# ueda0319/neddf

Hardware: NVIDIA H100
Metric: ray-samples/s (800x800x192) (higher is better)
Workload: dtype f16x3-split operands, f32 accumulate

## Files before the change

### neddf_b200/csrc/composite.cu

```cuda
#include "common.cuh"

namespace neddf {

constexpr int kWarpsPerBlock = 8;

__global__ void __launch_bounds__(kWarpsPerBlock * 32)
composite_kernel(const float* __restrict__ dists, const float* __restrict__ density,
                 const float* __restrict__ color, const float* __restrict__ penalty, int64_t n_rays,
                 int n_edges, float max_dist, float* __restrict__ weight, float* __restrict__ depth,
                 float* __restrict__ color_out, float* __restrict__ transmittance,
                 float* __restrict__ penalty_out, int* __restrict__ status) {
  const int lane = threadIdx.x & 31;
  const int64_t warp = (int64_t)blockIdx.x * kWarpsPerBlock + (threadIdx.x >> 5);
  const int64_t n_warps = (int64_t)gridDim.x * kWarpsPerBlock;
  const int n_int = n_edges - 1;
  bool saw_nan = false;

  for (int64_t ray = warp; ray < n_rays; ray += n_warps) {
    const float* drow = dists + ray * n_edges;
    const float* srow = density + ray * n_edges;
    const float* crow = color + ray * n_edges * 3;
    const float* prow = penalty ? penalty + ray * n_edges : nullptr;
    float* wrow = weight ? weight + ray * n_int : nullptr;

    double carry = 1.0;
    float acc_d = 0.f, acc_r = 0.f, acc_g = 0.f, acc_b = 0.f, acc_p = 0.f;
    for (int base = 0; base < n_int; base += 32) {
      const int j = base + lane;
      const bool live = j < n_int;
      float dj = 0.f, delta = 0.f, o = 0.f;
      if (live) {
        dj = drow[j];
        delta = drow[j + 1] - dj;
        o = 1.0f - (float)exp((double)(-srow[j] * delta));
      }
      double f = live ? (double)(1.0f - o + 1e-7f) : 1.0;
      double incl = f;
#pragma unroll
      for (int s = 1; s < 32; s <<= 1) {
        double up = __shfl_up_sync(0xffffffffu, incl, s);
        if (lane >= s) incl *= up;
      }
      double excl = __shfl_up_sync(0xffffffffu, incl, 1);
      if (lane == 0) excl = 1.0;
      float t_j = (float)(carry * excl);
      if (live) {
        float w = o * t_j;
        saw_nan |= (w != w);
        if (wrow) wrow[j] = w;
        acc_d += w * dj;
        acc_r += w * crow[3 * j + 0];
        acc_g += w * crow[3 * j + 1];
        acc_b += w * crow[3 * j + 2];
        if (prow) acc_p += delta * prow[j];
      }
      carry = carry * __shfl_sync(0xffffffffu, incl, 31);
    }
#pragma unroll
    for (int s = 16; s > 0; s >>= 1) {
      acc_d += __shfl_xor_sync(0xffffffffu, acc_d, s);
      acc_r += __shfl_xor_sync(0xffffffffu, acc_r, s);
      acc_g += __shfl_xor_sync(0xffffffffu, acc_g, s);
      acc_b += __shfl_xor_sync(0xffffffffu, acc_b, s);
      acc_p += __shfl_xor_sync(0xffffffffu, acc_p, s);
    }
    if (lane == 0) {
      float t_last = (float)carry;
      if (depth) depth[ray] = acc_d + t_last * max_dist;
      if (color_out) {
        color_out[3 * ray + 0] = acc_r;
        color_out[3 * ray + 1] = acc_g;
        color_out[3 * ray + 2] = acc_b;
      }
      if (transmittance) transmittance[ray] = t_last;
      if (penalty_out) penalty_out[ray] = acc_p;
    }
  }
  if (status && __any_sync(0xffffffffu, saw_nan) && lane == 0) atomicOr(status, 1);
}

__global__ void __launch_bounds__(kWarpsPerBlock * 32)
composite_backward_kernel(const float* __restrict__ dists, const float* __restrict__ density,
                          const float* __restrict__ color, int64_t n_rays, int n_edges, float max_dist,
                          const float* __restrict__ g_weight, const float* __restrict__ g_depth,
                          const float* __restrict__ g_color, const float* __restrict__ g_trans,
                          const float* __restrict__ g_pen, float* __restrict__ d_density,
// ... 95 lines not shown

}

using namespace neddf;

extern "C" int32_t neddf_composite_backward(const float* d_dists, const float* d_density, const float* d_color,
                                            int64_t n_rays, int32_t n_edges, float max_dist, const float* g_weight,
                                            const float* g_depth, const float* g_color, const float* g_transmittance,
                                            const float* g_penalty, float* d_grad_density, float* d_grad_color,
                                            float* d_grad_penalty, void* stream) {
  if (n_rays < 0 || n_edges < 2) return fail(NEDDF_E_INVALID, "neddf_composite_backward: bad sizes");
  if (n_rays == 0) return NEDDF_OK;
  if (!d_dists || !d_density || !d_color) return fail(NEDDF_E_INVALID, "neddf_composite_backward: null input pointer");
  size_t smem = (size_t)kWarpsPerBlock * 2 * (n_edges - 1) * sizeof(float);
  if (smem > 200 * 1024) return fail(NEDDF_E_UNSUPPORTED, "neddf_composite_backward: too many samples per ray");
  if (smem > 48 * 1024)
    NEDDF_CUDA_CHECK(cudaFuncSetAttribute(composite_backward_kernel, cudaFuncAttributeMaxDynamicSharedMemorySize, (int)smem));
  int64_t blocks = (n_rays + kWarpsPerBlock - 1) / kWarpsPerBlock;
  int64_t cap = (int64_t)sm_count() * 8;
  if (blocks > cap) blocks = cap;
  composite_backward_kernel<<<(unsigned)blocks, kWarpsPerBlock * 32, smem, (cudaStream_t)stream>>>(
      d_dists, d_density, d_color, n_rays, n_edges, max_dist, g_weight, g_depth, g_color, g_transmittance, g_penalty,
      d_grad_density, d_grad_color, d_grad_penalty);
  NEDDF_LAUNCH_CHECK();
  return NEDDF_OK;
}

extern "C" int32_t neddf_composite(const float* d_dists, const float* d_density, const float* d_color,
                                   const float* d_penalty, int64_t n_rays, int32_t n_edges, float max_dist,
                                   float* d_weight, float* d_depth, float* d_color_out, float* d_transmittance,
                                   float* d_penalty_out, int32_t* d_status, void* stream) {
  if (n_rays < 0 || n_edges < 1) return fail(NEDDF_E_INVALID, "neddf_composite: bad sizes");
  if (n_rays == 0) return NEDDF_OK;
  if (!d_dists || !d_density || !d_color) return fail(NEDDF_E_INVALID, "neddf_composite: null input pointer");
  if (d_penalty_out && !d_penalty) return fail(NEDDF_E_INVALID, "neddf_composite: penalty_out without penalty");
  int64_t blocks = (n_rays + kWarpsPerBlock - 1) / kWarpsPerBlock;
  int64_t cap = (int64_t)sm_count() * 8;
  if (blocks > cap) blocks = cap;
  composite_kernel<<<(unsigned)blocks, kWarpsPerBlock * 32, 0, (cudaStream_t)stream>>>(
      d_dists, d_density, d_color, d_penalty_out ? d_penalty : nullptr, n_rays, n_edges, max_dist, d_weight,
      d_depth, d_color_out, d_transmittance, d_penalty_out, d_status);
  NEDDF_LAUNCH_CHECK();
  return NEDDF_OK;
}


namespace neddf {
__global__ void terminate_rays_kernel(const float* __restrict__ dists, const float* __restrict__ density, int n_edges,
                                      int edge0, int seg_len, const int32_t* __restrict__ idx_in,
                                      const int32_t* __restrict__ n_in, int64_t n_rays, float* __restrict__ trans,
                                      float eps, int32_t* __restrict__ idx_out, int32_t* __restrict__ n_out,
                                      unsigned long long* __restrict__ executed) {
  const int64_t count = idx_in ? (int64_t)(*n_in) : n_rays;
  if (executed && blockIdx.x == 0 && threadIdx.x == 0) atomicAdd(executed, (unsigned long long)(count * seg_len));
  for (int64_t i0 = (int64_t)blockIdx.x * blockDim.x; i0 < count; i0 += (int64_t)gridDim.x * blockDim.x) {
    const int64_t i = i0 + threadIdx.x;
    bool keep = false;
    int32_t ray = 0;
    if (i < count) {
      ray = idx_in ? idx_in[i] : (int32_t)i;
      const float* d = dists + (int64_t)ray * n_edges;
      const float* s = density + (int64_t)ray * n_edges;
      float t = trans[ray];
      const int e1 = min(edge0 + seg_len, n_edges - 1);
      for (int j = edge0; j < e1; ++j) {
        const float o = 1.0f - expf(-s[j] * (d[j + 1] - d[j]));
        t *= (1.0f - o + 1e-7f);
// ... 35 lines not shown
```

### neddf_b200/csrc/field_tc.cu

```cuda
#include "tc_ptx.cuh"

#include <algorithm>
#include <cstring>

namespace neddf {
namespace tc {

constexpr int kStages = 3;
constexpr int kConsumers = 256;
constexpr int kConsumerWarps = kConsumers / 32;
constexpr int kThreads = kConsumers + 128;
constexpr uint32_t kConsumerRegs = 232, kProducerRegs = 40;

constexpr uint32_t kOffHHi = 0;
constexpr uint32_t kOffHLo = kOffHHi + kHBytes;
constexpr uint32_t kOffAuxHi = kOffHLo + kHBytes;
constexpr uint32_t kOffAuxLo = kOffAuxHi + kAuxBytes;
constexpr uint32_t kOffRing = kOffAuxLo + kAuxBytes;
constexpr uint32_t kOffScratch = kOffRing + kStages * kChunkBytes;

struct Scratch {
  float geo[kTileS][12];
  uint64_t full[kStages];
  uint64_t empty[kStages];
};
constexpr uint32_t kSmemBytes = kOffScratch + sizeof(Scratch);
static_assert(kSmemBytes <= 227 * 1024, "shared memory budget");

constexpr int kGroup = kRows / kTileS;
constexpr uint32_t kParkH = kHBytes / kGroup, kParkAux = kAuxBytes / kGroup;
constexpr uint32_t kParkBytes = 2 * kParkH + 2 * kParkAux;

struct TcLayer {
  int aux_ksteps;
  int h_ksteps;
};

struct TcParams {
  FieldParams f;
  TcLayer layer[kMaxHidden];
  int chunks_per_tile;
  int dist_chunks;
  const unsigned char* w_tc;
  const float* bias;
  int* status;
  int eval;
  unsigned char* park;
};

__device__ __forceinline__ uint32_t cluster_ctarank() {
  uint32_t r;
  asm volatile("mov.u32 %0, %%cluster_ctarank;" : "=r"(r));
  return r;
}
__device__ __forceinline__ void cluster_sync_all() {
  asm volatile("barrier.cluster.arrive.release.aligned;\nbarrier.cluster.wait.acquire.aligned;" ::: "memory");
}
__device__ __forceinline__ uint32_t mapa_u32(uint32_t saddr, uint32_t rank) {
  uint32_t r;
  asm volatile("mapa.shared::cluster.u32 %0, %1, %2;" : "=r"(r) : "r"(saddr), "r"(rank));
  return r;
}
__device__ __forceinline__ void mbar_arrive_remote(uint32_t caddr) {
  asm volatile("mbarrier.arrive.release.cluster.shared::cluster.b64 _, [%0];" ::"r"(caddr) : "memory");
}
__device__ __forceinline__ void mbar_wait_cluster(uint64_t* bar, uint32_t parity) {
  asm volatile(
      "{\n"
      ".reg .pred p;\n"
      "TC_WAITC:\n"
      "mbarrier.try_wait.parity.acquire.cluster.shared::cta.b64 p, [%0], %1;\n"
      "@p bra TC_DONEC;\n"
      "bra TC_WAITC;\n"
      "TC_DONEC:\n"
      "}\n" ::"r"(smem_u32(bar)),
      "r"(parity)
      : "memory");
}
__device__ __forceinline__ void tma_bulk_g2s_pair(uint32_t dst_smem, const void* src, uint32_t bytes, uint64_t* bar) {
// ... 92 lines not shown
      ph_t = now_;                         \
    }                                      \
  } while (0)
#else
#define TC_PHASE(i) \
  do {              \
  } while (0)
#endif

template <int ACT, bool PAIR>
__global__ void __launch_bounds__(kThreads, 1) field_tc_kernel(const __grid_constant__ TcParams P) {
  extern __shared__ __align__(1024) unsigned char smem[];
  const FieldParams& p = P.f;
  unsigned char* h_hi = smem + kOffHHi;
  unsigned char* h_lo = smem + kOffHLo;
  unsigned char* aux_hi = smem + kOffAuxHi;
  unsigned char* aux_lo = smem + kOffAuxLo;
  unsigned char* ring = smem + kOffRing;
  Scratch* sc = reinterpret_cast<Scratch*>(smem + kOffScratch);

  const int tid = threadIdx.x;
  const int warp = tid >> 5, lane = tid & 31;
  const int n_hidden = p.n_ddf + p.n_col;

  const int64_t n_total = field_total(p);
  const int64_t n_tiles = (n_total + kTileS - 1) / kTileS;
  const uint32_t rank = PAIR ? cluster_ctarank() : 0;
  const int64_t unit = PAIR ? (int64_t)(blockIdx.x >> 1) : (int64_t)blockIdx.x;
  const int64_t n_units = PAIR ? (int64_t)(gridDim.x >> 1) : (int64_t)gridDim.x;
  const int64_t units_total = PAIR ? (n_tiles + 1) / 2 : n_tiles;
  int64_t my_tiles = 0;
  if (unit < units_total) my_tiles = (units_total - 1 - unit) / n_units + 1;
  auto tile_of = [&](int64_t t) { return PAIR ? 2 * (unit + t * n_units) + rank : unit + t * n_units; };
  const int group = P.eval ? kGroup : 1;

  if (tid == 0) {
    for (int i = 0; i < kStages; ++i) {
      mbar_init(&sc->full[i], 1);
      mbar_init(&sc->empty[i], PAIR ? 2 * kConsumerWarps : kConsumerWarps);
    }
    asm volatile("fence.mbarrier_init.release.cluster;" ::: "memory");
  }
  __syncthreads();
  if (PAIR) cluster_sync_all();

  if (warp >= kConsumerWarps) {
    asm volatile("setmaxnreg.dec.sync.aligned.u32 %0;" ::"n"(kProducerRegs));
    if (warp == kConsumerWarps && lane == 0) {
      int64_t g = 0;
      auto push = [&](int c) {
        const int s = (int)(g % kStages);
        if (g >= kStages) mbar_wait_cluster(&sc->empty[s], (uint32_t)((g / kStages - 1) & 1));
        mbar_expect_tx(&sc->full[s], kChunkBytes);
        const unsigned char* src = P.w_tc + (size_t)c * kChunkBytes;
        const uint32_t dst = smem_u32(ring + s * kChunkBytes);
        if (PAIR) tma_bulk_g2s_pair(dst + rank * (kChunkBytes / 2), src + rank * (kChunkBytes / 2), kChunkBytes / 2, &sc->full[s]);
        else tma_bulk_g2s(dst, src, kChunkBytes, &sc->full[s]);
        ++g;
      };
      for (int64_t base = 0; base < my_tiles; base += group) {
        const int gn = (int)std::min<int64_t>(group, my_tiles - base);
        for (int i = 0; i < gn; ++i)
          for (int c = 0; c < P.dist_chunks; ++c) push(c);
        for (int c = P.dist_chunks; c < P.chunks_per_tile; ++c) push(c);
      }
    }
  } else {
    asm volatile("setmaxnreg.inc.sync.aligned.u32 %0;" ::"n"(kConsumerRegs));
    const int wg = tid >> 7;
    const int chb = 128 * wg + 16 * ((tid & 127) >> 5) + (lane >> 2);
    const int cq = 2 * (lane & 3);
    const int hs = tid >> 3, hj = (tid >> 1) & 3, hk = tid & 1;
    const int hbase = lane & ~7;
    float bad = 0.f;
    __half2 badh = __floats2half2_rn(0.f, 0.f);
    uint32_t peer_empty[kStages];
#pragma unroll
    for (int i = 0; i < kStages; ++i) peer_empty[i] = PAIR ? mapa_u32(smem_u32(&sc->empty[i]), rank ^ 1) : 0u;
    auto release = [&](int64_t g) {
      if (lane == 0) {
        const int s = (int)(g % kStages);
        mbar_arrive(&sc->empty[s]);
        if (PAIR) mbar_arrive_remote(peer_empty[s]);
      }
    };
    int64_t g = 0;
    HeadOut head;
    std::memset(&head, 0, sizeof(head));
#ifdef NEDDF_TC_PHASE_CLOCKS
    long long ph_sum[kPhCount] = {}, ph_t = clock64();
#endif

    unsigned char* park = P.park + (size_t)blockIdx.x * kGroup * kParkBytes;

    auto layer = [&](int l, int64_t base, int gn) {
      const int64_t n0 = tile_of(base) * kTileS;
      const TcLayer L = P.layer[l];
// ... 96 lines not shown
      TC_PHASE(l < p.n_ddf ? kPhDistance : kPhColour);

      const int hrow = 32 * hj + hs;
      const uint32_t hrow_off = (uint32_t)((hrow >> 3) * (kHK * 16) + (hrow & 7) * 2);
      const int rot = hj + 4 * hk;
      auto hval = [&](int k) {
        return __half2float(*reinterpret_cast<const __half*>(h_hi + hrow_off + k * 16)) +
               __half2float(*reinterpret_cast<const __half*>(h_lo + hrow_off + k * 16));
      };
      if (l == p.n_ddf - 1) {
        float pd = 0.f, pa = 0.f;
#pragma unroll 4
        for (int kk = 0; kk < 128; ++kk) {
          const int k = 128 * hk + ((kk + rot) & 127);
          const float v = hval(k);
          const float2 wv = __ldg(reinterpret_cast<const float2*>(p.w_head_da) + k);
          pd = fmaf(v, wv.x, pd);
          pa = fmaf(v, wv.y, pa);
        }
        pd += __shfl_xor_sync(0xffffffffu, pd, 1);
        pa += __shfl_xor_sync(0xffffffffu, pa, 1);
        float ddf[4], aux[4];
#pragma unroll
        for (int j = 0; j < 4; ++j) {
          ddf[j] = __shfl_sync(0xffffffffu, pd, hbase + 2 * j);
          aux[j] = __shfl_sync(0xffffffffu, pa, hbase + 2 * j);
        }
        const int rows = P.eval ? 1 : 4;
        if (hj == 0 && hk == 0) {
          ddf[0] += __ldg(p.b_head + 0);
          aux[0] += __ldg(p.b_head + 1);
          head_density(ddf, aux, p.d_near, p.aux_grad_scale, p.density_act, head);
          const int kn = p.n_e0 + p.n_d;
#pragma unroll
          for (int c = 0; c < 3; ++c) store_sample(aux_hi, aux_lo, kAuxK, hs, kn + c, head.normal[c], 0.f, 0.f, 0.f, bad, rows);
          const int64_t n = n0 + hs;
          if (n < n_total) {
            int64_t ray_, on;
            int j_;
            field_map(p, n, ray_, j_, on);
            if (p.distance) p.distance[on] = head.distance;
            if (p.density) p.density[on] = head.density;
            if (p.aux_grad) p.aux_grad[on] = head.aux;
          }
        }
        {
          const int s = tid >> 3, sub = tid & 7;
          write_pos_embedding(p, sc->geo, aux_hi, aux_lo, s, sub, 8, false, bad, rows);
          const int dhalf = 3 * p.embed_dir;
          for (int idx = sub; idx < dhalf; idx += 8) {
            int e = idx / 3, d = idx - 3 * e;
            float sn, cs;
            sincosf((float)(1u << e) * sc->geo[s][3 + d], &sn, &cs);
            store_sample(aux_hi, aux_lo, kAuxK, s, p.n_e0 + idx, sn, 0.f, 0.f, 0.f, bad, rows);
            store_sample(aux_hi, aux_lo, kAuxK, s, p.n_e0 + dhalf + idx, cs, 0.f, 0.f, 0.f, bad, rows);
          }
          for (int k = p.n_e0 + p.n_d + 3 + sub; k < kAuxK; k += 8)
            store_sample(aux_hi, aux_lo, kAuxK, s, k, 0.f, 0.f, 0.f, 0.f, bad, rows);
        }
        bar_consumers();
      } else if (l == n_hidden - 1) {
        if (cgroup) {
          const int row = tid >> 1, ck = tid & 1;
          const uint32_t row_off = (uint32_t)((row >> 3) * (kHK * 16) + (row & 7) * 2);
          float pc[3] = {0.f, 0.f, 0.f};
#pragma unroll 4
          for (int kk = 0; kk < 128; ++kk) {
            const int k = 128 * ck + ((kk + 4 * ck) & 127);
            const float v = __half2float(*reinterpret_cast<const __half*>(h_hi + row_off + k * 16)) +
                            __half2float(*reinterpret_cast<const __half*>(h_lo + row_off + k * 16));
            const float4 wv = __ldg(reinterpret_cast<const float4*>(p.w_head_col) + k);
            pc[0] = fmaf(v, wv.x, pc[0]);
            pc[1] = fmaf(v, wv.y, pc[1]);
            pc[2] = fmaf(v, wv.z, pc[2]);
          }
#pragma unroll
          for (int c = 0; c < 3; ++c) pc[c] += __shfl_xor_sync(0xffffffffu, pc[c], 1);
          const int64_t n = tile_of(base + (row >> 5)) * kTileS + (row & 31);
          if (ck == 0 && (row >> 5) < gn && n < n_total && p.color) {
// ... 35 lines not shown
            field_map(p, n, ray_, j_, on);
            if (p.color) {
              p.color[3 * on + 0] = col[0];
              p.color[3 * on + 1] = col[1];
              p.color[3 * on + 2] = col[2];
            }
            if (p.penalty) p.penalty[on] = field_penalty(head, col, colJ, p.distance_range_max, p.penalty_weight);
          }
        }
      }
      fence_async_smem();
      bar_consumers();
      TC_PHASE(l == p.n_ddf - 1 || l == n_hidden - 1 ? kPhHeads : l < p.n_ddf ? kPhDistance : kPhColour);
    };

    for (int64_t base = 0; base < my_tiles; base += group) {
      const int gn = (int)std::min<int64_t>(group, my_tiles - base);
      for (int gi = 0; gi < gn; ++gi) {
        const int64_t n0 = tile_of(base + gi) * kTileS;
        if (tid < kTileS) tile_geometry(p, sc->geo, n0, tid, n_total);
        bar_consumers();
        {
          const int s = tid >> 3, sub = tid & 7;
          write_pos_embedding(p, sc->geo, aux_hi, aux_lo, s, sub, 8, true, bad);
          for (int k = p.n_e0 + sub; k < 64; k += 8) store_sample(aux_hi, aux_lo, kAuxK, s, k, 0.f, 0.f, 0.f, 0.f, bad);
        }
        fence_async_smem();
        bar_consumers();
        TC_PHASE(kPhPrologue);
#ifdef NEDDF_TC_PHASE_CLOCKS
        if (tid == 0) ++ph_sum[kPhTiles];
#endif
        for (int l = 0; l < p.n_ddf; ++l) layer(l, base + gi, 1);
        if (P.eval) {
          park_move<false>(smem, park + gi * kParkBytes, 0, tid);
          TC_PHASE(kPhPark);
        }
      }
      if (P.eval) {
        bar_consumers();
        for (int j = 0; j < kGroup; ++j) park_move<true>(smem, j < gn ? park + j * kParkBytes : nullptr, j, tid);
        fence_async_smem();
        bar_consumers();
        TC_PHASE(kPhPark);
      }
      for (int l = p.n_ddf; l < n_hidden; ++l) layer(l, base, gn);
    }
#ifdef NEDDF_TC_PHASE_CLOCKS
    if (tid == 0)
      for (int i = 0; i < kPhCount; ++i) atomicAdd(&g_tc_phase[i], (unsigned long long)ph_sum[i]);
#endif
    const float2 m = __half22float2(badh);
    if (!(fmaxf(bad, fmaxf(m.x, m.y)) < 65504.0f) && P.status) atomicOr(P.status, 4);
  }
  if (PAIR) cluster_sync_all();
}

struct TcPackArgs {
  const float* w[kMaxHidden];
  const float* b[kMaxHidden];
  int k_in[kMaxHidden];
  int aux_real[kMaxHidden];
  int aux_pad[kMaxHidden];
  int ksteps[kMaxHidden];
  int chunk0[kMaxHidden];
  int n_hidden;
};

__global__ void tc_pack_hidden_kernel(TcPackArgs a, unsigned char* __restrict__ dst, float* __restrict__ bias) {
  const int l = blockIdx.y;
  const int total = a.ksteps[l] * kWidth * 16;
// ... 144 lines not shown
  cudaFree(S->d_status);
  cudaFree(S->d_park);
  delete S;
  f->tc = nullptr;
}

int32_t tc_pack_weights(neddf_field* f, const float* const* d_w, const float* const* d_b, cudaStream_t s) {
  int32_t rc = tc_ensure(f);
  if (rc != NEDDF_OK) return rc;
  tc::TcStorage* S = static_cast<tc::TcStorage*>(f->tc);
  tc::TcPackArgs a = S->pack;
  const int n_hidden = f->n_ddf + f->n_col;
  for (int l = 0; l < n_hidden; ++l) {
    a.w[l] = d_w[l];
    a.b[l] = d_b[l];
  }
  tc::tc_pack_hidden_kernel<<<dim3(64, n_hidden), 256, 0, s>>>(a, S->d_w, S->d_bias);
  NEDDF_LAUNCH_CHECK();
  return NEDDF_OK;
}

int32_t launch_field_tc(const neddf_field* f, FieldParams& p, int flags, bool pair, cudaStream_t s) {
  tc::TcStorage* S = static_cast<tc::TcStorage*>(f->tc);
  if (!S) return fail(NEDDF_E_INVALID, "tensor-core engine: weights were never packed");
  tc::TcParams P;
  P.f = p;
  for (int l = 0; l < p.n_ddf + p.n_col; ++l) P.layer[l] = S->layer[l];
  P.chunks_per_tile = S->chunks_per_tile;
  P.dist_chunks = S->dist_chunks;
  P.w_tc = S->d_w;
  P.bias = S->d_bias;
  P.status = S->d_status;
  P.eval = (flags == NEDDF_OUT_EVAL && p.penalty == nullptr && p.save_pre == nullptr) ? 1 : 0;
  if (P.eval && !S->d_park) {
    if (cudaMalloc(&S->d_park, (size_t)sm_count() * tc::kGroup * tc::kParkBytes) != cudaSuccess) {
      S->d_park = nullptr;
      return fail(NEDDF_E_CUDA, "tensor-core engine: cudaMalloc of the colour-trunk scratch failed");
    }
  }
  P.park = S->d_park;
  const int64_t n_tiles = (p.n + tc::kTileS - 1) / tc::kTileS;
  auto launch = [&](auto kern) -> int32_t {
    NEDDF_CUDA_CHECK(cudaFuncSetAttribute(kern, cudaFuncAttributeMaxDynamicSharedMemorySize, (int)tc::kSmemBytes));
    cudaLaunchConfig_t cfg = {};
    cudaLaunchAttribute attr[1];
    cfg.blockDim = dim3(tc::kThreads);
    cfg.dynamicSmemBytes = tc::kSmemBytes;
    cfg.stream = s;
    if (pair) {
      const int64_t pairs = (n_tiles + 1) / 2;
      cfg.gridDim = dim3((unsigned)(2 * std::max<int64_t>(1, std::min<int64_t>(pairs, sm_count() / 2))));
      attr[0].id = cudaLaunchAttributeClusterDimension;
      attr[0].val.clusterDim.x = 2;
      attr[0].val.clusterDim.y = 1;
      attr[0].val.clusterDim.z = 1;
      cfg.attrs = attr;
      cfg.numAttrs = 1;
    } else {
      cfg.gridDim = dim3((unsigned)std::max<int64_t>(1, std::min<int64_t>(n_tiles, sm_count())));
      cfg.numAttrs = 0;
    }
    NEDDF_CUDA_CHECK(cudaLaunchKernelEx(&cfg, kern, P));
    NEDDF_LAUNCH_CHECK();
    return NEDDF_OK;
  };
  switch (p.hidden_act) {
    case NEDDF_ACT_TANHEXP: return pair ? launch(tc::field_tc_kernel<NEDDF_ACT_TANHEXP, true>) : launch(tc::field_tc_kernel<NEDDF_ACT_TANHEXP, false>);
// ... 45 lines not shown
```

### neddf_b200/nerf.py

```python
import math
import os
from typing import Dict, List, Optional

import torch
from torch import Tensor, nn

from . import _lib as L
from ._host import KernelHandle, WeightGrad
from .network import BaseNeuralField
from .ray import Sampling


def lowpass_scale(embed_dim: int, alpha: float) -> List[float]:
    if alpha >= embed_dim:
        return [1.0] * embed_dim
    s = [1.0] * embed_dim
    k = int(alpha)
    s[k] = 0.5 * (1.0 - math.cos(math.pi * (alpha - k))) + 1e-7
    for i in range(k + 1, embed_dim):
        s[i] = 1e-7
    return s


class _NerfTrainFn(torch.autograd.Function):
# ... 119 lines not shown
        c.density_activation_type = L.ACT_IDS[self.density_activation_type]
        return self._fill_skips(c)

    def _launch_forward(self, a: Tensor, b: Tensor, c: Tensor, sampling_type, ray_radius: float) -> Dict[str, Tensor]:
        if sampling_type is not None:
            return self.forward_rays(a, b, c, sampling_type, ray_radius)
        return self.forward(Sampling(a, b, c))

    def _forward_autograd(self, a: Tensor, b: Tensor, c: Tensor, sampling_type, ray_radius: float) -> Dict[str, Tensor]:
        density, color = _NerfTrainFn.apply(self, a, b, c, sampling_type, float(ray_radius), *self._param_tensors())
        return {"density": density, "color": color}

    def _lowpass(self):
        return L.fbuf(lowpass_scale(self.embed_pos_rank, self.lowpass_alpha))

    def forward(self, sampling: Sampling) -> Dict[str, Tensor]:
        pos = L.require_cuda_f32(sampling.sample_pos, "sample_pos")
        sdir = L.require_cuda_f32(sampling.sample_dir, "sample_dir")
        var = L.require_cuda_f32(sampling.diag_variance, "diag_variance")
        B, S = pos.shape[0], pos.shape[1]
        if self._wants_grad():
            return self._forward_autograd(pos.reshape(B, S, 3), sdir.reshape(B, S, 3), var.reshape(B, S, 3), None, 0.0)
        device = pos.device
        out = {"density": torch.empty(B, S, device=device, dtype=torch.float32),
               "color": torch.empty(B, S, 3, device=device, dtype=torch.float32)}
        h = self._field(device)
        with torch.cuda.device(device):
            L.check(L.lib().neddf_nerf_forward(h, self._lowpass(), L.ptr(pos), L.ptr(sdir), L.ptr(var), B * S,
                                               L.ptr(out["density"]), L.ptr(out["color"]), L.stream_ptr(device)),
                    "nerf_forward")
        return out

    def forward_rays(self, ray_dir: Tensor, ray_orig: Tensor, dists: Tensor, sampling_type: str, ray_radius: float,
                     need_penalty: bool = True, need_aux: bool = True) -> Dict[str, Tensor]:
        ray_dir = L.require_cuda_f32(ray_dir, "ray_dir")
        ray_orig = L.require_cuda_f32(ray_orig, "ray_orig")
        dists = L.require_cuda_f32(dists, "dists")
        if self._wants_grad():
            return self._forward_autograd(ray_dir, ray_orig, dists, sampling_type, ray_radius)
        B, S = dists.shape
        device = dists.device
        out = {"density": torch.empty(B, S, device=device, dtype=torch.float32),
               "color": torch.empty(B, S, 3, device=device, dtype=torch.float32)}
        h = self._field(device)
        with self._profiled(device, B * S), torch.cuda.device(device):
            L.check(L.lib().neddf_nerf_forward_rays(h, self._lowpass(), L.ptr(ray_dir), L.ptr(ray_orig), L.ptr(dists), B, S,
                                                    L.SAMPLING_IDS[sampling_type], float(ray_radius), L.ptr(out["density"]),
                                                    L.ptr(out["color"]), L.stream_ptr(device)), "nerf_forward_rays")
        return out

    def set_iter(self, iter: int) -> None:
        if iter == -1:
            self.lowpass_alpha = float(self.embed_pos_rank)
        else:
            self.lowpass_alpha = self.lowpass_alpha_offset + 0.001 * iter
```

### neddf_b200/network.py

```python
import contextlib
import ctypes as C
import warnings
from typing import Dict, List, Optional, Tuple

import numpy as np
import torch
from torch import Tensor, nn

from . import _lib as L
from ._host import KernelHandle, WeightGrad
from .ray import Sampling


class LinearGradLayer(nn.Module):

    def __init__(self, input_ch: int = 128, output_ch: int = 128) -> None:
        super().__init__()
        self.input_ch, self.output_ch = input_ch, output_ch
        self.weight = nn.Parameter(torch.randn(input_ch, output_ch))
        self.bias = nn.Parameter(torch.randn(output_ch))
        nn.init.xavier_normal_(self.weight)
        nn.init.constant_(self.bias, 0.0)

    def forward(self, *a, **k):
# ... 438 lines not shown
        return L.FieldState(float(self.aux_grad_scale), float(self.distance_range_max), float(self.lowpass_alpha), pw)

    def forward(self, sampling: Sampling) -> Dict[str, Tensor]:
        pos = sampling.sample_pos
        B, S = pos.shape[0], pos.shape[1]
        if self._wants_grad():
            p3 = L.require_cuda_f32(pos.reshape(B, S, 3), "sample_pos")
            d3 = L.require_cuda_f32(sampling.sample_dir.reshape(B, S, 3), "sample_dir")
            v3 = L.require_cuda_f32(sampling.diag_variance.reshape(B, S, 3), "diag_variance")
            d, c, pnl, dist, aux = _FieldTrainFn.apply(self, p3, d3, v3, None, 0.0, *self._param_tensors())
            return {"distance": dist, "density": d, "color": c, "fields_penalty": pnl, "aux_grad": aux}
        device = pos.device
        p3 = L.require_cuda_f32(pos.reshape(-1, 3), "sample_pos")
        d3 = L.require_cuda_f32(sampling.sample_dir.reshape(-1, 3), "sample_dir")
        v3 = L.require_cuda_f32(sampling.diag_variance.reshape(-1, 3), "diag_variance")
        n = B * S
        out = {
            "distance": torch.empty(B, S, device=device, dtype=torch.float32),
            "density": torch.empty(B, S, device=device, dtype=torch.float32),
            "color": torch.empty(B, S, 3, device=device, dtype=torch.float32),
            "fields_penalty": torch.empty(B, S, device=device, dtype=torch.float32),
            "aux_grad": torch.empty(B, S, device=device, dtype=torch.float32),
        }
        h = self._field(device)
        st = self._state_struct()
        with torch.cuda.device(device):
            L.check(L.lib().neddf_field_forward(
                h, C.byref(st), L.ptr(p3), L.ptr(d3), L.ptr(v3), n, L.ptr(out["distance"]), L.ptr(out["density"]),
                L.ptr(out["color"]), L.ptr(out["fields_penalty"]), L.ptr(out["aux_grad"]), L.OUT_FULL,
                self._engine_id(), L.stream_ptr(device)), "field_forward")
        return out

    def forward_rays(self, ray_dir: Tensor, ray_orig: Tensor, dists: Tensor, sampling_type: str, ray_radius: float,
                     need_penalty: bool = True, need_aux: bool = True) -> Dict[str, Tensor]:
        ray_dir = L.require_cuda_f32(ray_dir, "ray_dir")
        ray_orig = L.require_cuda_f32(ray_orig, "ray_orig")
        dists = L.require_cuda_f32(dists, "dists")
        if self._wants_grad():
            d, c, pnl = _FieldTrainFn.apply(self, ray_dir, ray_orig, dists, sampling_type, ray_radius,
                                            *self._param_tensors())
            return {"density": d, "color": c, "fields_penalty": pnl}
        B, S = dists.shape
        device = dists.device
        out = {
            "density": torch.empty(B, S, device=device, dtype=torch.float32),
            "color": torch.empty(B, S, 3, device=device, dtype=torch.float32),
        }
        if need_penalty:
            out["fields_penalty"] = torch.empty(B, S, device=device, dtype=torch.float32)
        if need_aux:
            out["distance"] = torch.empty(B, S, device=device, dtype=torch.float32)
            out["aux_grad"] = torch.empty(B, S, device=device, dtype=torch.float32)
        h = self._field(device)
        st = self._state_struct()
        with self._profiled(device, B * S), torch.cuda.device(device):
            L.check(L.lib().neddf_field_forward_rays(
                h, C.byref(st), L.ptr(ray_dir), L.ptr(ray_orig), L.ptr(dists), B, S, L.SAMPLING_IDS[sampling_type],
                float(ray_radius), L.ptr(out.get("distance")), L.ptr(out["density"]), L.ptr(out["color"]),
                L.ptr(out.get("fields_penalty")), L.ptr(out.get("aux_grad")),
                L.OUT_FULL if need_penalty else L.OUT_EVAL, self._engine_id(), L.stream_ptr(device)),
                "field_forward_rays")
        return out

    def forward_rays_segment(self, ray_dir: Tensor, ray_orig: Tensor, dists: Tensor, sampling_type: str, ray_radius: float,
                             edge0: int, seg_len: int, ray_index: Optional[Tensor], n_active: Optional[Tensor],
                             density: Tensor, color: Tensor) -> None:
        B, E = dists.shape
        device = dists.device
        h = self._field(device)
        st = self._state_struct()
        with self._profiled(device, None), torch.cuda.device(device):
            L.check(L.lib().neddf_field_forward_rays_segment(
                h, C.byref(st), L.ptr(ray_dir), L.ptr(ray_orig), L.ptr(dists), B, E, L.SAMPLING_IDS[sampling_type],
                float(ray_radius), int(edge0), int(seg_len), L.ptr(ray_index), L.ptr(n_active), L.ptr(density),
                L.ptr(color), self._engine_id(), L.stream_ptr(device)), "field_forward_rays_segment")

    def check_engine_status(self) -> None:
        if self._handle is None:
            return
        v = C.c_int32(0)
        dev = self._handle_device
        with torch.cuda.device(dev):
            L.check(L.lib().neddf_field_status(self._handle, C.byref(v), L.stream_ptr(dev)), "field_status")
        if v.value & 4:
            if self.engine == "auto" and not self._range_fallback:
                self._range_fallback = True
                raise EngineRangeError(
                    "neddf_b200: tensor-core engine saw |activation| > 65504 (fp16 range of its split operands); "
                    "engine 'auto' now resolves to the fp32 engine for this network and the call is re-run")
            raise FloatingPointError(
                "neddf_b200: tensor-core engine saw |activation| > 65504 (fp16 range of its split operands); "
# ... 12 lines not shown
```

### neddf_b200/neus.py

```python
import ctypes as C
import os
from typing import Dict, List, Optional

import torch
from torch import Tensor, nn

from . import _lib as L
from ._host import KernelHandle, WeightGrad
from .network import BaseNeuralField
from .ray import Sampling


def unit_normals(g: Tensor) -> Tensor:
    return torch.nn.functional.normalize(g, dim=1)


class _NeusTrainFn(torch.autograd.Function):

    @staticmethod
    def forward(ctx, net, a, b, c, sampling_type, ray_radius, with_normal, *params):
        with torch.no_grad():
            out = net._launch_forward(a, b, c, sampling_type, ray_radius, with_normal)
        ctx.net, ctx.meta = net, (sampling_type, float(ray_radius))
        ctx.save_for_backward(a, b, c)
# ... 136 lines not shown
    def _shade_hits(self, hits: Tensor, pos: Tensor, dirs: Tensor, normal: Tensor, color: Tensor) -> None:
        p = pos[None]
        out = self.forward(Sampling(p, dirs[None], p), with_normal=True)
        idx = hits.long()
        normal.index_copy_(0, idx, unit_normals(out["normal"].reshape(-1, 3)))
        color.index_copy_(0, idx, out["color"].reshape(-1, 3))

    @staticmethod
    def _outputs(B: int, S: int, device, with_normal: bool) -> Dict[str, Tensor]:
        out = {"sdf": torch.empty(B, S, device=device, dtype=torch.float32),
               "density": torch.empty(B, S, device=device, dtype=torch.float32),
               "color": torch.empty(B, S, 3, device=device, dtype=torch.float32)}
        if with_normal:
            out["normal"] = torch.empty(B, S, 3, device=device, dtype=torch.float32)
        return out

    def forward(self, sampling: Sampling, with_normal: bool = False) -> Dict[str, Tensor]:
        wants_grad = self._wants_grad()
        pos = L.require_cuda_f32(sampling.sample_pos, "sample_pos")
        sdir = L.require_cuda_f32(sampling.sample_dir, "sample_dir")
        B, S = pos.shape[0], pos.shape[1]
        if wants_grad:
            return self._forward_autograd(pos.reshape(B, S, 3), sdir.reshape(B, S, 3), None, None, 0.0, with_normal)
        device = pos.device
        out = self._outputs(B, S, device, with_normal)
        h = self._field(device)
        with torch.cuda.device(device):
            L.check(L.lib().neddf_neus_forward(h, L.ptr(pos), L.ptr(sdir), B * S, L.ptr(out["sdf"]), L.ptr(out["density"]),
                                               L.ptr(out["color"]), L.ptr(out.get("normal")), L.stream_ptr(device)),
                    "neus_forward")
        return out

    def forward_rays(self, ray_dir: Tensor, ray_orig: Tensor, dists: Tensor, sampling_type: str, ray_radius: float,
                     need_penalty: bool = True, need_aux: bool = True, with_normal: bool = False) -> Dict[str, Tensor]:
        wants_grad = self._wants_grad()
        ray_dir = L.require_cuda_f32(ray_dir, "ray_dir")
        ray_orig = L.require_cuda_f32(ray_orig, "ray_orig")
        dists = L.require_cuda_f32(dists, "dists")
        if wants_grad:
            return self._forward_autograd(ray_dir, ray_orig, dists, sampling_type, ray_radius, with_normal)
        B, S = dists.shape
        device = dists.device
        out = self._outputs(B, S, device, with_normal)
        h = self._field(device)
        with self._profiled(device, B * S), torch.cuda.device(device):
            L.check(L.lib().neddf_neus_forward_rays(h, L.ptr(ray_dir), L.ptr(ray_orig), L.ptr(dists), B, S,
                                                    L.SAMPLING_IDS[sampling_type], float(ray_radius), L.ptr(out["sdf"]),
                                                    L.ptr(out["density"]), L.ptr(out["color"]), L.ptr(out.get("normal")),
                                                    L.stream_ptr(device)), "neus_forward_rays")
        return out
```

### neddf_b200/render.py

```python
import importlib
import math
import warnings
from typing import Any, Dict, Iterable, List, Optional, Tuple

import numpy as np
import torch
from torch import Tensor, nn

from . import _lib as L
from .nerf import NeRF
from .network import BaseNeuralField, EngineRangeError, NeDDF
from .neus import NeuS
from .ray import CONE_RAY_RADIUS, Ray

_TARGET_ALIASES = {
    "neddf.network.NeDDF": NeDDF,
    "neddf.network.neddf.NeDDF": NeDDF,
    "neddf_b200.NeDDF": NeDDF,
    "neddf_b200.network.NeDDF": NeDDF,
    "neddf.network.NeRF": NeRF,
    "neddf.network.nerf.NeRF": NeRF,
    "neddf_b200.NeRF": NeRF,
    "neddf_b200.nerf.NeRF": NeRF,
    "neddf.network.NeuS": NeuS,
# ... 86 lines not shown

    def __init__(self) -> None:
        super().__init__()
        self.iteration: int = -1

    def set_iter(self, iter: int) -> None:
        self.iteration = iter

    def next_iter(self) -> None:
        self.set_iter(self.iteration + 1)

    def sample_pdf(self, dists: Tensor, weights: Tensor, samples_fine: int, cat_coarse: bool = True,
                   uniform_rands: Optional[Tensor] = None, return_ids: bool = False):
        dists = L.require_cuda_f32(dists, "dists")
        if weights.dtype != torch.float32 or not weights.is_contiguous() or not weights.is_cuda:
            raise RuntimeError("neddf_b200: `weights` must be a contiguous fp32 CUDA tensor (it is updated in place)")
        B, E = dists.shape
        if weights.shape != (B, E - 1):
            raise ValueError(f"weights must be [batch, {E - 1}]")
        device = dists.device
        if uniform_rands is None:
            uniform_rands = torch.rand(B, samples_fine, device=device)
        u = L.require_cuda_f32(uniform_rands, "uniform_rands")
        if u.shape != (B, samples_fine):
            raise ValueError("uniform_rands must be [batch, samples_fine]")
        out = torch.empty(B, (E if cat_coarse else 0) + samples_fine, device=device, dtype=torch.float32)
        ids = torch.empty(B, samples_fine, device=device, dtype=torch.int64) if return_ids else None
        status = self._status(device)
        with torch.cuda.device(device):
            L.check(L.lib().neddf_sample_pdf(L.ptr(dists), L.ptr(weights), L.ptr(u), B, E, samples_fine, 1 if cat_coarse else 0, L.ptr(out),
                                             L.ptr(ids), None, L.ptr(status), L.stream_ptr(device)), "sample_pdf")
        return (out, ids) if return_ids else out

    def integrate_volume_render(self, dists: Tensor, densities: Tensor, colors: Tensor,
                                penalties: Optional[Tensor] = None) -> Dict[str, Tensor]:
        dists = L.require_cuda_f32(dists, "dists")
        densities = L.require_cuda_f32(densities, "densities")
        colors = L.require_cuda_f32(colors, "colors")
        B, E = dists.shape
        device = dists.device
        if torch.is_grad_enabled() and (densities.requires_grad or colors.requires_grad or
                                        (penalties is not None and penalties.requires_grad)):
            if penalties is not None:
                penalties = L.require_cuda_f32(penalties, "penalties")
            w, d, c, t, p_ = _CompositeFn.apply(dists.detach(), densities, colors, penalties, self.max_dist,
                                                self._status(device))
            res = {"weight": w, "depth": d, "color": c, "transmittance": t}
            if penalties is not None:
                res["fields_penalty"] = p_
            return res
        res = {
            "weight": torch.empty(B, E - 1, device=device, dtype=torch.float32),
            "depth": torch.empty(B, device=device, dtype=torch.float32),
            "color": torch.empty(B, 3, device=device, dtype=torch.float32),
            "transmittance": torch.empty(B, device=device, dtype=torch.float32),
        }
        pen_out = None
        if penalties is not None:
            penalties = L.require_cuda_f32(penalties, "penalties")
            pen_out = torch.empty(B, device=device, dtype=torch.float32)
        status = self._status(device)
        with torch.cuda.device(device):
            L.check(L.lib().neddf_composite(L.ptr(dists), L.ptr(densities), L.ptr(colors), L.ptr(penalties), B, E,
                                            float(self.max_dist), L.ptr(res["weight"]), L.ptr(res["depth"]),
                                            L.ptr(res["color"]), L.ptr(res["transmittance"]), L.ptr(pen_out),
                                            L.ptr(status), L.stream_ptr(device)), "composite")
        if pen_out is not None:
            res["fields_penalty"] = pen_out
        return res

    def _status(self, device) -> Tensor:
        st = getattr(self, "_status_buf", None)
        if st is None or st.device != device:
            st = torch.zeros(2, device=device, dtype=torch.int32)
            self._status_buf = st
        return st

    def check_status(self) -> None:
        range_error = None
        for net in {id(n): n for n in (getattr(self, "network_coarse", None), getattr(self, "network_fine", None))
                    if n is not None}.values():
            if hasattr(net, "check_engine_status"):
                try:
                    net.check_engine_status()
                except EngineRangeError as e:
                    range_error = e
        st = getattr(self, "_status_buf", None)
        if range_error is not None:
            if st is not None:
                st.zero_()
            raise range_error
        if st is None:
            return
        v = int(st[0].item())
        st.zero_()
        if v & 1:
            raise AssertionError("NaN in volume-rendering weights (base_neural_render.py:155)")
        if v & 2:
# ... 30 lines not shown
        self.sampling_type = sampling_type
        self.check_nan = True
        self.image_chunk = 163840
        self.transmittance_eps = 0.0
        self.termination_segments = 4
        self._term_counters = None

    def get_network(self) -> BaseNeuralField:
        return self.network_fine

    def get_parameters_list(self) -> List[Any]:
        if self.use_coarse_network:
            return list(self.network_coarse.parameters()) + list(self.network_fine.parameters())
        return list(self.network_coarse.parameters())

    def set_iter(self, iter: int) -> None:
        super().set_iter(iter)
        self.network_coarse.set_iter(iter)
        self.network_fine.set_iter(iter)

    def set_engine(self, engine: str) -> None:
        if engine not in L.ENGINE_IDS:
            raise ValueError(engine)
        for net in (self.network_fine, self.network_coarse):
            net.engine = engine
            if hasattr(net, "_range_fallback"):
                net._range_fallback = False

    @property
    def _ray_radius(self) -> float:
        return CONE_RAY_RADIUS if self.sampling_type == "cone" else 0.0

    def _render_core(self, ray_dir: Tensor, ray_orig: Tensor, u_coarse: Tensor, u_fine: Tensor,
                     full: bool) -> Dict[str, Tensor]:
        lib = L.lib()
        B = ray_dir.shape[0]
        device = ray_dir.device
        Ec, Ef_new = self.sample_coarse + 1, self.sample_fine + 1
        stream = L.stream_ptr(device)
        dists_c = torch.empty(B, Ec, device=device, dtype=torch.float32)
        L.check(lib.neddf_coarse_dists(L.ptr(u_coarse), B, Ec, self.dist_near, self.dist_far, L.ptr(dists_c), stream),
                "coarse_dists")
        vc = self.network_coarse.forward_rays(ray_dir, ray_orig, dists_c, self.sampling_type, self._ray_radius,
                                              need_penalty=full, need_aux=False)
        ic = self.integrate_volume_render(dists_c, vc["density"], vc["color"], vc.get("fields_penalty"))
        dists_f = self.sample_pdf(dists_c, ic["weight"], Ef_new, uniform_rands=u_fine)
        if (not full and self.transmittance_eps > 0.0 and not torch.is_grad_enabled()
                and hasattr(self.network_fine, "forward_rays_segment")):
            vf = self._fine_pass_terminated(ray_dir, ray_orig, dists_f)
        else:
            vf = self.network_fine.forward_rays(ray_dir, ray_orig, dists_f, self.sampling_type, self._ray_radius,
                                                need_penalty=full, need_aux=False)
        out = self.integrate_volume_render(dists_f, vf["density"], vf["color"], vf.get("fields_penalty"))
        for k in list(ic.keys()):
            out[k + "_coarse"] = ic[k]
        return out

    def _fine_pass_terminated(self, ray_dir: Tensor, ray_orig: Tensor, dists_f: Tensor) -> Dict[str, Tensor]:
        lib = L.lib()
        B, E = dists_f.shape
        device = dists_f.device
        density = torch.zeros(B, E, device=device, dtype=torch.float32)
        color = torch.zeros(B, E, 3, device=device, dtype=torch.float32)
        trans = torch.ones(B, device=device, dtype=torch.float32)
        idx = [torch.empty(B, device=device, dtype=torch.int32) for _ in range(2)]
        cnt = [torch.zeros(1, device=device, dtype=torch.int32) for _ in range(2)]
        if self._term_counters is None or self._term_counters.device != device:
            self._term_counters = torch.zeros(2, device=device, dtype=torch.int64)
        executed = self._term_counters[0:1]
        self._term_counters[1] += B * E
        K = max(1, min(int(self.termination_segments), E))
        bounds = [round(k * E / K) for k in range(K + 1)]
        cur_idx, cur_n = None, None
        stream = L.stream_ptr(device)
        for k in range(K):
            e0, seg = bounds[k], bounds[k + 1] - bounds[k]
            self.network_fine.forward_rays_segment(ray_dir, ray_orig, dists_f, self.sampling_type, self._ray_radius, e0, seg,
                                                   cur_idx, cur_n, density, color)
# ... 34 lines not shown
        with torch.cuda.device(device):
            ray_dir = torch.empty(B, 3, device=device, dtype=torch.float32)
            ray_orig = torch.empty(B, 3, device=device, dtype=torch.float32)
            L.check(L.lib().neddf_make_rays(L.ptr(uv), L.UV_DTYPES[uv.dtype], B, hR, hT, hC, L.ptr(ray_dir),
                                            L.ptr(ray_orig), L.stream_ptr(device)), "make_rays")
            u_c, u_f = self._uniforms(B, device, uniforms)
            out = self._render_core(ray_dir, ray_orig, u_c, u_f, full=True)
            if self.check_nan:
                try:
                    self.check_status()
                except EngineRangeError as e:
                    warnings.warn(str(e), RuntimeWarning)
                    out = None
                    out = self._render_core(ray_dir, ray_orig, u_c, u_f, full=True)
                    self.check_status()
        return out

    def create_rays(self, uv: Tensor, camera) -> Ray:
        uv = uv.contiguous()
        if uv.dtype not in L.UV_DTYPES:
            uv = uv.to(torch.int64)
        B, device = uv.shape[0], uv.device
        hR, hT, hC = _camera_host(camera)
        ray_dir = torch.empty(B, 3, device=device, dtype=torch.float32)
        ray_orig = torch.empty(B, 3, device=device, dtype=torch.float32)
        with torch.cuda.device(device):
            L.check(L.lib().neddf_make_rays(L.ptr(uv), L.UV_DTYPES[uv.dtype], B, hR, hT, hC, L.ptr(ray_dir),
                                            L.ptr(ray_orig), L.stream_ptr(device)), "make_rays")
        return Ray(ray_dir, ray_orig, uv)

    def render_pixels(self, width: int, height: int, camera, target_types: Iterable[str], downsampling: int,
                      first: int, count: int, uniforms=None, device=None) -> Dict[str, Tensor]:
        target_types = list(target_types)
        lib = L.lib()
        device = torch.device(device) if device is not None else self.network_fine.device
        if device.type != "cuda":
            raise RuntimeError(f"neddf_b200.NeRFRender renders on CUDA devices only (the module is on {device}): move it "
                               "with .to('cuda') - the hot path has no CPU implementation")
        hR, hT, hC = _camera_host(camera)
        outs: Dict[str, List[Tensor]] = {k: [] for k in target_types}
        with torch.no_grad(), torch.cuda.device(device):
            for b0 in range(first, first + count, self.image_chunk):
                n = min(self.image_chunk, first + count - b0)
                ray_dir = torch.empty(n, 3, device=device, dtype=torch.float32)
                ray_orig = torch.empty(n, 3, device=device, dtype=torch.float32)
                L.check(lib.neddf_make_image_rays(int(width), int(height), int(downsampling), b0, n, hR, hT, hC,
                                                  L.ptr(ray_dir), L.ptr(ray_orig), L.stream_ptr(device)),
                        "make_image_rays")
                if uniforms is None:
                    u = None
                else:
                    u = (uniforms[0][b0 - first:b0 - first + n], uniforms[1][b0 - first:b0 - first + n])
                u_c, u_f = self._uniforms(n, device, u)
                res = self._render_core(ray_dir, ray_orig, u_c, u_f, full=False)
                for k in target_types:
                    outs[k].append(res[k].reshape(n, -1))
        return {k: (torch.cat(v, 0) if len(v) != 1 else v[0]) for k, v in outs.items()}

    def render_image(self, width: int, height: int, camera, target_types: Iterable[str], downsampling: int = 1,
                     chunk: int = 512, uniforms=None) -> Dict[str, Tensor]:
        target_types = list(target_types)
        w, h = width // downsampling, height // downsampling
        was_training = (self.network_coarse.training, self.network_fine.training)
        self.network_coarse.eval()
        self.network_fine.eval()
        try:
            flat = self.render_pixels(width, height, camera, target_types, downsampling, 0, w * h, uniforms)
        finally:
            self.network_coarse.train(True)
            self.network_fine.train(True)
        del was_training
        if self.check_nan:
            try:
                self.check_status()
            except EngineRangeError as e:
                warnings.warn(str(e), RuntimeWarning)
                with torch.no_grad():
                    flat = self.render_pixels(width, height, camera, target_types, downsampling, 0, w * h, uniforms)
                self.check_status()
        return {k: v.reshape(h, w, -1) for k, v in flat.items()}

    def render_surface(self, width: int, height: int, camera, downsampling: int = 1, level: Optional[float] = None,
                       max_steps: int = 128) -> Dict[str, Tensor]:
        width, height, downsampling = (int(v) for v in (width, height, downsampling))
        if downsampling < 1 or width < downsampling or height < downsampling:
            raise ValueError(f"render_surface: need downsampling >= 1 and width, height >= downsampling, got "
                             f"{width}x{height} / {downsampling}")
# ... 45 lines not shown
```

Baseline: 30.23 million.

## Skip coarse-network colour branch when rendering only needs fine outputs

Adds a density-only mode to the tensor-core field kernel and lets colour be optional in compositing. When rendering pixels without coarse targets, the coarse pass no longer runs the colour trunk, its input embedding or the park/unpark staging, and the composite kernel skips colour accumulation. The goal is to drop the colour work that sampling only needs density for. The cost is extra branching and new optional-pointer paths through the Python and C APIs.

```diff
diff --git a/neddf_b200/csrc/composite.cu b/neddf_b200/csrc/composite.cu
--- a/neddf_b200/csrc/composite.cu
+++ b/neddf_b200/csrc/composite.cu
@@ -19,7 +19,7 @@
   for (int64_t ray = warp; ray < n_rays; ray += n_warps) {
     const float* drow = dists + ray * n_edges;
     const float* srow = density + ray * n_edges;
-    const float* crow = color + ray * n_edges * 3;
+    const float* crow = color ? color + ray * n_edges * 3 : nullptr;
     const float* prow = penalty ? penalty + ray * n_edges : nullptr;
     float* wrow = weight ? weight + ray * n_int : nullptr;
 
@@ -49,9 +49,11 @@
         saw_nan |= (w != w);
         if (wrow) wrow[j] = w;
         acc_d += w * dj;
-        acc_r += w * crow[3 * j + 0];
-        acc_g += w * crow[3 * j + 1];
-        acc_b += w * crow[3 * j + 2];
+        if (crow) {
+          acc_r += w * crow[3 * j + 0];
+          acc_g += w * crow[3 * j + 1];
+          acc_b += w * crow[3 * j + 2];
+        }
         if (prow) acc_p += delta * prow[j];
       }
       carry = carry * __shfl_sync(0xffffffffu, incl, 31);
@@ -213,7 +215,8 @@
                                    float* d_penalty_out, int32_t* d_status, void* stream) {
   if (n_rays < 0 || n_edges < 1) return fail(NEDDF_E_INVALID, "neddf_composite: bad sizes");
   if (n_rays == 0) return NEDDF_OK;
-  if (!d_dists || !d_density || !d_color) return fail(NEDDF_E_INVALID, "neddf_composite: null input pointer");
+  if (!d_dists || !d_density) return fail(NEDDF_E_INVALID, "neddf_composite: null input pointer");
+  if (d_color_out && !d_color) return fail(NEDDF_E_INVALID, "neddf_composite: color_out without color");
   if (d_penalty_out && !d_penalty) return fail(NEDDF_E_INVALID, "neddf_composite: penalty_out without penalty");
   int64_t blocks = (n_rays + kWarpsPerBlock - 1) / kWarpsPerBlock;
   int64_t cap = (int64_t)sm_count() * 8;
diff --git a/neddf_b200/csrc/field_tc.cu b/neddf_b200/csrc/field_tc.cu
--- a/neddf_b200/csrc/field_tc.cu
+++ b/neddf_b200/csrc/field_tc.cu
@@ -45,6 +45,7 @@
   const float* bias;
   int* status;
   int eval;
+  int density_only;
   unsigned char* park;
 };
 
@@ -203,7 +204,8 @@
   int64_t my_tiles = 0;
   if (unit < units_total) my_tiles = (units_total - 1 - unit) / n_units + 1;
   auto tile_of = [&](int64_t t) { return PAIR ? 2 * (unit + t * n_units) + rank : unit + t * n_units; };
-  const int group = P.eval ? kGroup : 1;
+  const int group = P.eval && !P.density_only ? kGroup : 1;
+  const int chunks_end = P.density_only ? P.dist_chunks : P.chunks_per_tile;
 
   if (tid == 0) {
     for (int i = 0; i < kStages; ++i) {
@@ -233,7 +235,7 @@
         const int gn = (int)std::min<int64_t>(group, my_tiles - base);
         for (int i = 0; i < gn; ++i)
           for (int c = 0; c < P.dist_chunks; ++c) push(c);
-        for (int c = P.dist_chunks; c < P.chunks_per_tile; ++c) push(c);
+        for (int c = P.dist_chunks; c < chunks_end; ++c) push(c);
       }
     }
   } else {
@@ -396,8 +398,10 @@
           aux[0] += __ldg(p.b_head + 1);
           head_density(ddf, aux, p.d_near, p.aux_grad_scale, p.density_act, head);
           const int kn = p.n_e0 + p.n_d;
-#pragma unroll
-          for (int c = 0; c < 3; ++c) store_sample(aux_hi, aux_lo, kAuxK, hs, kn + c, head.normal[c], 0.f, 0.f, 0.f, bad, rows);
+          if (!P.density_only) {
+#pragma unroll
+            for (int c = 0; c < 3; ++c) store_sample(aux_hi, aux_lo, kAuxK, hs, kn + c, head.normal[c], 0.f, 0.f, 0.f, bad, rows);
+          }
           const int64_t n = n0 + hs;
           if (n < n_total) {
             int64_t ray_, on;
@@ -408,7 +412,7 @@
             if (p.aux_grad) p.aux_grad[on] = head.aux;
           }
         }
-        {
+        if (!P.density_only) {
           const int s = tid >> 3, sub = tid & 7;
           write_pos_embedding(p, sc->geo, aux_hi, aux_lo, s, sub, 8, false, bad, rows);
           const int dhalf = 3 * p.embed_dir;
@@ -510,11 +514,12 @@
         if (tid == 0) ++ph_sum[kPhTiles];
 #endif
         for (int l = 0; l < p.n_ddf; ++l) layer(l, base + gi, 1);
-        if (P.eval) {
+        if (P.eval && !P.density_only) {
           park_move<false>(smem, park + gi * kParkBytes, 0, tid);
           TC_PHASE(kPhPark);
         }
       }
+      if (P.density_only) continue;
       if (P.eval) {
         bar_consumers();
         for (int j = 0; j < kGroup; ++j) park_move<true>(smem, j < gn ? park + j * kParkBytes : nullptr, j, tid);
@@ -725,7 +730,8 @@
   P.bias = S->d_bias;
   P.status = S->d_status;
   P.eval = (flags == NEDDF_OUT_EVAL && p.penalty == nullptr && p.save_pre == nullptr) ? 1 : 0;
-  if (P.eval && !S->d_park) {
+  P.density_only = (p.color == nullptr && p.penalty == nullptr && p.save_pre == nullptr) ? 1 : 0;
+  if (P.eval && !P.density_only && !S->d_park) {
     if (cudaMalloc(&S->d_park, (size_t)sm_count() * tc::kGroup * tc::kParkBytes) != cudaSuccess) {
       S->d_park = nullptr;
       return fail(NEDDF_E_CUDA, "tensor-core engine: cudaMalloc of the colour-trunk scratch failed");
diff --git a/neddf_b200/nerf.py b/neddf_b200/nerf.py
--- a/neddf_b200/nerf.py
+++ b/neddf_b200/nerf.py
@@ -175,7 +175,7 @@
         return out
 
     def forward_rays(self, ray_dir: Tensor, ray_orig: Tensor, dists: Tensor, sampling_type: str, ray_radius: float,
-                     need_penalty: bool = True, need_aux: bool = True) -> Dict[str, Tensor]:
+                     need_penalty: bool = True, need_aux: bool = True, need_color: bool = True) -> Dict[str, Tensor]:
         ray_dir = L.require_cuda_f32(ray_dir, "ray_dir")
         ray_orig = L.require_cuda_f32(ray_orig, "ray_orig")
         dists = L.require_cuda_f32(dists, "dists")
diff --git a/neddf_b200/network.py b/neddf_b200/network.py
--- a/neddf_b200/network.py
+++ b/neddf_b200/network.py
@@ -494,7 +494,7 @@
         return out
 
     def forward_rays(self, ray_dir: Tensor, ray_orig: Tensor, dists: Tensor, sampling_type: str, ray_radius: float,
-                     need_penalty: bool = True, need_aux: bool = True) -> Dict[str, Tensor]:
+                     need_penalty: bool = True, need_aux: bool = True, need_color: bool = True) -> Dict[str, Tensor]:
         ray_dir = L.require_cuda_f32(ray_dir, "ray_dir")
         ray_orig = L.require_cuda_f32(ray_orig, "ray_orig")
         dists = L.require_cuda_f32(dists, "dists")
@@ -504,10 +504,9 @@
             return {"density": d, "color": c, "fields_penalty": pnl}
         B, S = dists.shape
         device = dists.device
-        out = {
-            "density": torch.empty(B, S, device=device, dtype=torch.float32),
-            "color": torch.empty(B, S, 3, device=device, dtype=torch.float32),
-        }
+        out = {"density": torch.empty(B, S, device=device, dtype=torch.float32)}
+        if need_color or need_penalty:
+            out["color"] = torch.empty(B, S, 3, device=device, dtype=torch.float32)
         if need_penalty:
             out["fields_penalty"] = torch.empty(B, S, device=device, dtype=torch.float32)
         if need_aux:
@@ -518,7 +517,7 @@
         with self._profiled(device, B * S), torch.cuda.device(device):
             L.check(L.lib().neddf_field_forward_rays(
                 h, C.byref(st), L.ptr(ray_dir), L.ptr(ray_orig), L.ptr(dists), B, S, L.SAMPLING_IDS[sampling_type],
-                float(ray_radius), L.ptr(out.get("distance")), L.ptr(out["density"]), L.ptr(out["color"]),
+                float(ray_radius), L.ptr(out.get("distance")), L.ptr(out["density"]), L.ptr(out.get("color")),
                 L.ptr(out.get("fields_penalty")), L.ptr(out.get("aux_grad")),
                 L.OUT_FULL if need_penalty else L.OUT_EVAL, self._engine_id(), L.stream_ptr(device)),
                 "field_forward_rays")
diff --git a/neddf_b200/neus.py b/neddf_b200/neus.py
--- a/neddf_b200/neus.py
+++ b/neddf_b200/neus.py
@@ -192,7 +192,7 @@
         return out
 
     def forward_rays(self, ray_dir: Tensor, ray_orig: Tensor, dists: Tensor, sampling_type: str, ray_radius: float,
-                     need_penalty: bool = True, need_aux: bool = True, with_normal: bool = False) -> Dict[str, Tensor]:
+                     need_penalty: bool = True, need_aux: bool = True, need_color: bool = True, with_normal: bool = False) -> Dict[str, Tensor]:
         wants_grad = self._wants_grad()
         ray_dir = L.require_cuda_f32(ray_dir, "ray_dir")
         ray_orig = L.require_cuda_f32(ray_orig, "ray_orig")
diff --git a/neddf_b200/render.py b/neddf_b200/render.py
--- a/neddf_b200/render.py
+++ b/neddf_b200/render.py
@@ -142,14 +142,18 @@
                                              L.ptr(ids), None, L.ptr(status), L.stream_ptr(device)), "sample_pdf")
         return (out, ids) if return_ids else out
 
-    def integrate_volume_render(self, dists: Tensor, densities: Tensor, colors: Tensor,
+    def integrate_volume_render(self, dists: Tensor, densities: Tensor, colors: Optional[Tensor],
                                 penalties: Optional[Tensor] = None) -> Dict[str, Tensor]:
         dists = L.require_cuda_f32(dists, "dists")
         densities = L.require_cuda_f32(densities, "densities")
-        colors = L.require_cuda_f32(colors, "colors")
+        if colors is None:
+            if torch.is_grad_enabled() and densities.requires_grad:
+                raise ValueError("integrate_volume_render: colors=None has no backward")
+        else:
+            colors = L.require_cuda_f32(colors, "colors")
         B, E = dists.shape
         device = dists.device
-        if torch.is_grad_enabled() and (densities.requires_grad or colors.requires_grad or
+        if torch.is_grad_enabled() and (densities.requires_grad or (colors is not None and colors.requires_grad) or
                                         (penalties is not None and penalties.requires_grad)):
             if penalties is not None:
                 penalties = L.require_cuda_f32(penalties, "penalties")
@@ -162,9 +166,10 @@
         res = {
             "weight": torch.empty(B, E - 1, device=device, dtype=torch.float32),
             "depth": torch.empty(B, device=device, dtype=torch.float32),
-            "color": torch.empty(B, 3, device=device, dtype=torch.float32),
             "transmittance": torch.empty(B, device=device, dtype=torch.float32),
         }
+        if colors is not None:
+            res["color"] = torch.empty(B, 3, device=device, dtype=torch.float32)
         pen_out = None
         if penalties is not None:
             penalties = L.require_cuda_f32(penalties, "penalties")
@@ -173,7 +178,7 @@
         with torch.cuda.device(device):
             L.check(L.lib().neddf_composite(L.ptr(dists), L.ptr(densities), L.ptr(colors), L.ptr(penalties), B, E,
                                             float(self.max_dist), L.ptr(res["weight"]), L.ptr(res["depth"]),
-                                            L.ptr(res["color"]), L.ptr(res["transmittance"]), L.ptr(pen_out),
+                                            L.ptr(res.get("color")), L.ptr(res["transmittance"]), L.ptr(pen_out),
                                             L.ptr(status), L.stream_ptr(device)), "composite")
         if pen_out is not None:
             res["fields_penalty"] = pen_out
@@ -270,7 +275,7 @@
         return CONE_RAY_RADIUS if self.sampling_type == "cone" else 0.0
 
     def _render_core(self, ray_dir: Tensor, ray_orig: Tensor, u_coarse: Tensor, u_fine: Tensor,
-                     full: bool) -> Dict[str, Tensor]:
+                     full: bool, coarse_color: bool = True) -> Dict[str, Tensor]:
         lib = L.lib()
         B = ray_dir.shape[0]
         device = ray_dir.device
@@ -280,8 +285,8 @@
         L.check(lib.neddf_coarse_dists(L.ptr(u_coarse), B, Ec, self.dist_near, self.dist_far, L.ptr(dists_c), stream),
                 "coarse_dists")
         vc = self.network_coarse.forward_rays(ray_dir, ray_orig, dists_c, self.sampling_type, self._ray_radius,
-                                              need_penalty=full, need_aux=False)
-        ic = self.integrate_volume_render(dists_c, vc["density"], vc["color"], vc.get("fields_penalty"))
+                                              need_penalty=full, need_aux=False, need_color=full or coarse_color)
+        ic = self.integrate_volume_render(dists_c, vc["density"], vc.get("color"), vc.get("fields_penalty"))
         dists_f = self.sample_pdf(dists_c, ic["weight"], Ef_new, uniform_rands=u_fine)
         if (not full and self.transmittance_eps > 0.0 and not torch.is_grad_enabled()
                 and hasattr(self.network_fine, "forward_rays_segment")):
@@ -382,6 +387,7 @@
     def render_pixels(self, width: int, height: int, camera, target_types: Iterable[str], downsampling: int,
                       first: int, count: int, uniforms=None, device=None) -> Dict[str, Tensor]:
         target_types = list(target_types)
+        coarse_color = any(k.endswith("_coarse") for k in target_types)
         lib = L.lib()
         device = torch.device(device) if device is not None else self.network_fine.device
         if device.type != "cuda":
@@ -402,7 +408,7 @@
                 else:
                     u = (uniforms[0][b0 - first:b0 - first + n], uniforms[1][b0 - first:b0 - first + n])
                 u_c, u_f = self._uniforms(n, device, u)
-                res = self._render_core(ray_dir, ray_orig, u_c, u_f, full=False)
+                res = self._render_core(ray_dir, ray_orig, u_c, u_f, full=False, coarse_color=coarse_color)
                 for k in target_types:
                     outs[k].append(res[k].reshape(n, -1))
         return {k: (torch.cat(v, 0) if len(v) != 1 else v[0]) for k, v in outs.items()}
```

After: 31.26 million, median of 6. 1.03x the previous value.
